# rarimo/ultragroth

Measured on AMD Instinct MI355X. Metric: proofs/s, higher is better.
Workload: dtype u32x9 (29-bit limbs, 254-bit modular integers)

## Files before the change

### ultragroth_amd/csrc/internal.hpp

```cpp
#pragma once
#include <hip/hip_runtime.h>
#include <cstdint>
#include <cstddef>
#include <vector>
#include "ec.hpp"
#include "stream_timer.hpp"

namespace ug {

Fr fr_root_of_unity(int s);
void bitrev_copy(u32* out, const u32* in, int logn, hipStream_t stream);

struct NttFusion {
    const u32* in2 = nullptr; u32* work = nullptr; const u32* fin_a = nullptr; const u32* fin_b = nullptr;
    u64 in2_stride = 0, work_stride = 0, fin_a_stride = 0, fin_b_stride = 0;
};

struct NttPass {
    const u32* in; u32* out; const u32* tw; const u32* post; const u32* post_const; const u32* in2; const u32* fin_a; const u32* fin_b;
    int logn, s0, k, j, gather_bitrev, scatter_bitrev;
    u64 in_stride, out_stride, in2_stride, fin_a_stride, fin_b_stride;
};
constexpr int NTT_MAX_PASSES = 8;

// ... 52 lines not shown
    void set_classes(const BucketClasses& k);
    void set_vectors(int v, u64 stride);
    u64 vector_count() const { return n / (u64)vectors; }
    int window_sets() const { return tables ? stride : windows; }
    int class_sets() const { return cls.on() ? (int)cls.cnt : 1; }
    int bucket_windows() const { return window_sets() * class_sets() * vectors; }
    u64 special_buckets() const { return cls.on() ? (u64)window_sets() * cls.specials : 0; }
    u64 total_buckets() const { return (u64)bucket_windows() * buckets + special_buckets(); }
    int result_points() const { return cls.on() ? 2 * bucket_windows() + (cls.specials ? window_sets() : 0) : bucket_windows(); }
    u64 expected_entries() const { return cls.on() ? ((n * (u64)windows) >> cls.q_log) * cls.cnt : n * (u64)windows; }
    DigitPlan digit_plan() const {
        DigitPlan d;
        d.n = n; d.c = c; d.windows = windows; d.buckets = buckets; d.sentinel = (u32)total_buckets(); d.tables = tables ? 1 : 0;
        d.set_map = 0; d.table_map = 0;
        if (tables)
            for (int w = 0; w < windows && w < 16; w++) { d.set_map |= (u64)(w % stride) << (4 * w); d.table_map |= (u64)(w / stride) << (4 * w); }
        d.q_log = cls.q_log; d.r0 = cls.r0; d.cnt = cls.on() ? cls.cnt : 1; d.specials = cls.on() ? cls.specials : 0;
        d.sp_lo = cls.sp_lo; d.sp_hi = cls.sp_hi; d.special_base = (u32)((u64)bucket_windows() * buckets);
        d.vec_count = (u32)vector_count(); d.vec_magic = 0; d.vec_shift = 0; d.vec_sets = (u32)window_sets(); d.vec_stride = vec_stride;
        if (vectors > 1) {
            int l = 0;
            while (((u64)1 << l) < (u64)d.vec_count) l++;
            d.vec_magic = (u32)((((u64)1 << 32) * (((u64)1 << l) - d.vec_count)) / d.vec_count + 1);
            d.vec_shift = l;
        }
        return d;
    }
};
constexpr int MSM_MAX_VECTORS = 16;
constexpr int TABLE_INDEX_BITS = 27;
constexpr int TABLE_MIN_C = 16, TABLE_MAX_C = 24;
double msm_model_cost(u64 n, int c, bool tables, int stride = 1);

struct HeavyBucket { u32 bucket, first_seg, last_seg, pad; };

int radix_plan(int bits, int* shift, int* bins_log);
void digit_pairs(const u32* scalars, const DigitPlan& plan, u32* keys, u32* vals, hipStream_t stream);
struct RadixSorter {
    u32* lookback = nullptr;
    u32* small = nullptr;
    u64 tiles_cap = 0;
    void reserve(u64 n_pairs, int ipt_min);
    void release();
    int sort(const u32* scalars, const MsmGeometry& geo, u32 sentinel, u64 n_pairs, int bits,
             u32* const buf_keys[2], u32* const buf_vals[2], u32* error_flag, hipStream_t stream, u32* n_valid_out = nullptr,
             bool* dropped_out = nullptr);
    ~RadixSorter() { release(); }
};

struct MsmSchedule {
    MsmGeometry geo;
    const u32* keys = nullptr;
    const u32* vals = nullptr;
    const u32* tkeys = nullptr;
    const u32* tvals = nullptr;
    u32* bucket_start = nullptr;
    u32* bucket_count = nullptr;
    u32* small_list = nullptr;
    int log_seg = 0;
    int log_seg_tail = 0;
    u32* heavy_list = nullptr;
    u32 heavy_cap = 0;
    u32* medium_list = nullptr;
    u32* heavy_offsets = nullptr;
    u32* meta = nullptr;
    u32 *keys_a = nullptr, *keys_b = nullptr, *vals_a = nullptr, *vals_b = nullptr;
    void* sort_tmp = nullptr; size_t sort_tmp_bytes = 0;
    RadixSorter sorter;
    u64 capacity_n = 0; u64 capacity_buckets = 0;
    void reserve(const MsmGeometry& g);
    void build(const u32* scalars_dev, const MsmGeometry& g, hipStream_t stream);
    void release();
    ~MsmSchedule() { release(); }
};

struct MsmWorkspace {
    u32* bucket_pts = nullptr;
    u32* chunk_pts = nullptr;
    u32* chunk_pts2 = nullptr;
    u32* slot_pts = nullptr;
    u32* task_pts = nullptr;
    size_t bucket_bytes = 0, chunk_bytes = 0, slot_bytes = 0, task_bytes = 0;
    void reserve(const MsmGeometry& g, bool g2, u64 n_segments, u32 n_heavy_tasks, int sets = 1);
    void release();
    ~MsmWorkspace() { release(); }
};

struct MsmPending {
    bool g2 = false;
    bool empty = true;
    int c = 0, window_sets = 0, class_sets = 1;
    int vectors = 1;
    BucketClasses cls;
    u32* host = nullptr;
};
constexpr int MSM_G2_PT_WORDS = 72;
constexpr size_t MSM_PENDING_WORDS = 128 * 72;
constexpr int MSM_QUEUE_DEPTH = 8;
constexpr int MSM_BATCH_WIDTH = 4;
struct MsmCall {
    struct Product { const u32* bases = nullptr; u64 n_bases = 0; int64_t delta = 0; u32* host = nullptr; };
    int count = 0;
    Product products[MSM_BATCH_WIDTH];
    int group = 0;
};
constexpr int MSM_PHASE_ALL = 0, MSM_PHASE_ACCUMULATE = 1, MSM_PHASE_TAIL = 2;
void msm_enqueue(bool g2, const MsmSchedule& s, MsmWorkspace& ws, const MsmCall& call, hipStream_t stream, LaunchTimer stats, MsmPending* pend,
                 int phase = MSM_PHASE_ALL);
// ... 61 lines not shown
```

### ultragroth_amd/csrc/msm.hip

```cpp
#ifdef UG_MEASURE
#include <hipcub/hipcub.hpp>
#endif
#include <algorithm>
#include <atomic>
#include <cstdlib>
#include <cstring>
#include <string>
#include <type_traits>
#include "dev_common.hpp"
#include "internal.hpp"
#include "segmap.hpp"

namespace ug {

namespace {

constexpr int LOG_SEG = 7;
constexpr u32 FIX_MAX = 32;
constexpr u32 MEDIUM_MAX = 4096;
constexpr u32 HEAVY_TASK = 1024;
constexpr int CHUNK = 32;

constexpr int ACC_BLOCK = 256;

typedef __attribute__((address_space(3))) u32 lds_u32;
template <class P> __device__ __forceinline__ void lds_get(Fp<P>& r, const lds_u32* p) {
#pragma unroll
    for (int i = 0; i < NL; i++) r.l[i] = p[i * ACC_BLOCK];
}
template <class P> __device__ __forceinline__ void lds_get(Fp2<P>& r, const lds_u32* p) { lds_get(r.a, p); lds_get(r.b, p + NL * ACC_BLOCK); }
template <class P> __device__ __forceinline__ void lds_set(lds_u32* p, const Fp<P>& v) {
#pragma unroll
    for (int i = 0; i < NL; i++) p[i * ACC_BLOCK] = v.l[i];
}
template <class P> __device__ __forceinline__ void lds_set(lds_u32* p, const Fp2<P>& v) { lds_set(p, v.a); lds_set(p + NL * ACC_BLOCK, v.b); }
template <class P> __device__ __forceinline__ u32 last_limb(const Fp<P>& v) { return v.l[NL - 1]; }
template <class P> __device__ __forceinline__ u32 last_limb(const Fp2<P>& v) { return v.b.l[NL - 1]; }
template <class F> struct TailLds {
    static constexpr int WORDS = sizeof(F) / sizeof(u32);
    static constexpr int AREA_WORDS = 2 * WORDS * ACC_BLOCK;
    lds_u32* slot;
    __device__ __forceinline__ lds_u32* after(const F& v) const {
        lds_u32* p = slot;
#if defined(__HIP_DEVICE_COMPILE__)
        asm volatile("" : "+v"(p) : "v"(last_limb(v)));
#endif
        return p;
    }
    __device__ __forceinline__ F zz() const { F r; lds_get(r, slot); return r; }
    __device__ __forceinline__ F zzz() const { F r; lds_get(r, slot + WORDS * ACC_BLOCK); return r; }
    __device__ __forceinline__ F zz_after(const F& v) const { F r; lds_get(r, after(v)); return r; }
    __device__ __forceinline__ F zzz_after(const F& v) const { F r; lds_get(r, after(v) + WORDS * ACC_BLOCK); return r; }
    __device__ __forceinline__ bool is_inf() const { return limbs_all_zero(zz()); }
    __device__ __forceinline__ void put(const F& zz, const F& zzz) { lds_set(slot, zz); lds_set(slot + WORDS * ACC_BLOCK, zzz); }
};

struct G1Cfg {
    typedef Fq F;
    typedef TailRegs<F> AccTail;
    static constexpr int AFF_WORDS = 16, PT_WORDS = 36, BLOCK = 256, ACC_WAVES = 3;
    static constexpr bool PREFETCH = true;
    static __device__ __forceinline__ bool load_affine(const u32* p, F& x, F& y) {
        u32 w[16];
        load8(w, p); load8(w + 8, p + 8);
        u32 o = 0;
#pragma unroll
        for (int i = 0; i < 16; i++) o |= w[i];
        if (o == 0) return false;
        x = unpack256<FqParams>(w); y = unpack256<FqParams>(w + 8);
        return true;
    }
    static __device__ __forceinline__ bool decode_affine(const u32* w, F& x, F& y) {
        u32 o = 0;
#pragma unroll
        for (int i = 0; i < 16; i++) o |= w[i];
        if (o == 0) return false;
        x = unpack256<FqParams>(w); y = unpack256<FqParams>(w + 8);
        return true;
    }
    static __device__ __forceinline__ void load_raw(u32* w, const u32* p) { load8(w, p); load8(w + 8, p + 8); }
    static __host__ __device__ __forceinline__ void store_affine_mont256(u32* o, const F& x, const F& y) {
        to_mont256(o, x); to_mont256(o + 8, y);
    }
    static __host__ __device__ __forceinline__ void store_affine_packed(u32* o, const F& x, const F& y) {
        pack256(o, cond_sub_q(mul(x, fp_one<FqParams>()))); pack256(o + 8, cond_sub_q(mul(y, fp_one<FqParams>())));
    }
    static __host__ __device__ __forceinline__ void to_words(u32* p, const XYZZ<F>& a, size_t stride) {
#pragma unroll
        for (int i = 0; i < NL; i++) {
            p[(size_t)i * stride] = a.x.l[i]; p[(size_t)(NL + i) * stride] = a.y.l[i];
            p[(size_t)(2 * NL + i) * stride] = a.zz.l[i]; p[(size_t)(3 * NL + i) * stride] = a.zzz.l[i];
        }
    }
    static __host__ __device__ __forceinline__ XYZZ<F> from_words(const u32* p, size_t stride) {
        XYZZ<F> a;
#pragma unroll
        for (int i = 0; i < NL; i++) {
            a.x.l[i] = p[(size_t)i * stride]; a.y.l[i] = p[(size_t)(NL + i) * stride];
            a.zz.l[i] = p[(size_t)(2 * NL + i) * stride]; a.zzz.l[i] = p[(size_t)(3 * NL + i) * stride];
        }
        return a;
    }
};
struct G2Cfg {
    typedef Fq2 F;
    typedef TailLds<F> AccTail;
    static constexpr int AFF_WORDS = 32, PT_WORDS = 72, BLOCK = 128, ACC_WAVES = 2;
    static constexpr bool PREFETCH = false;
    static __device__ __forceinline__ bool load_affine(const u32* p, F& x, F& y) {
        u32 w[32];
        load8(w, p); load8(w + 8, p + 8); load8(w + 16, p + 16); load8(w + 24, p + 24);
        u32 o = 0;
#pragma unroll
        for (int i = 0; i < 32; i++) o |= w[i];
        if (o == 0) return false;
        x.a = unpack256<FqParams>(w); x.b = unpack256<FqParams>(w + 8);
        y.a = unpack256<FqParams>(w + 16); y.b = unpack256<FqParams>(w + 24);
        return true;
    }
    static __device__ __forceinline__ bool decode_affine(const u32* w, F& x, F& y) {
        u32 o = 0;
#pragma unroll
        for (int i = 0; i < 32; i++) o |= w[i];
        if (o == 0) return false;
        x.a = unpack256<FqParams>(w); x.b = unpack256<FqParams>(w + 8);
        y.a = unpack256<FqParams>(w + 16); y.b = unpack256<FqParams>(w + 24);
        return true;
    }
    static __device__ __forceinline__ void load_raw(u32* w, const u32* p) {
        load8(w, p); load8(w + 8, p + 8); load8(w + 16, p + 16); load8(w + 24, p + 24);
    }
    static __host__ __device__ __forceinline__ void store_affine_mont256(u32* o, const F& x, const F& y) {
        to_mont256(o, x.a); to_mont256(o + 8, x.b); to_mont256(o + 16, y.a); to_mont256(o + 24, y.b);
    }
    static __host__ __device__ __forceinline__ void store_affine_packed(u32* o, const F& x, const F& y) {
        const Fq* f[4] = {&x.a, &x.b, &y.a, &y.b};
        for (int k = 0; k < 4; k++) pack256(o + 8 * k, cond_sub_q(mul(*f[k], fp_one<FqParams>())));
    }
    static __host__ __device__ __forceinline__ void to_words(u32* p, const XYZZ<F>& a, size_t stride) {
        const Fq* f[8] = {&a.x.a, &a.x.b, &a.y.a, &a.y.b, &a.zz.a, &a.zz.b, &a.zzz.a, &a.zzz.b};
#pragma unroll
        for (int k = 0; k < 8; k++)
#pragma unroll
            for (int i = 0; i < NL; i++) p[(size_t)(k * NL + i) * stride] = f[k]->l[i];
    }
    static __host__ __device__ __forceinline__ XYZZ<F> from_words(const u32* p, size_t stride) {
        XYZZ<F> a;
        Fq* f[8] = {&a.x.a, &a.x.b, &a.y.a, &a.y.b, &a.zz.a, &a.zz.b, &a.zzz.a, &a.zzz.b};
#pragma unroll
        for (int k = 0; k < 8; k++)
#pragma unroll
            for (int i = 0; i < NL; i++) f[k]->l[i] = p[(size_t)(k * NL + i) * stride];
        return a;
    }
};


__global__ void bucket_bounds_kernel(const u32* keys, u64 total_bound, u32 sentinel, u32* start, u32* count, u32* meta, int known) {
    const u64 total = known ? (u64)meta[1] : total_bound;
    const u64 p0 = ((u64)blockIdx.x * blockDim.x + threadIdx.x) * 4;
// ... 6 lines not shown
        for (int i = 0; i < 4; i++) k[1 + i] = p0 + i < total ? keys[p0 + i] : sentinel;
    }
    k[0] = p0 ? keys[p0 - 1] : sentinel;
    k[5] = p0 + 4 < total ? keys[p0 + 4] : sentinel;
#pragma unroll
    for (int i = 0; i < 4; i++) {
        const u64 p = p0 + i;
        const u32 key = k[1 + i];
        if (p >= total || key == sentinel) continue;
        if (p == 0 || k[i] != key) start[key] = (u32)p;
        if (k[2 + i] != key) count[key] = (u32)p + 1;
        if (k[2 + i] == sentinel) meta[1] = (u32)p + 1;
    }
}
__global__ __launch_bounds__(1024) void bucket_counts_kernel(u32* start, u32* count, u32 nb, int log_a, int log_b, u32* meta, u32* heavy_list,
                                                           u32* medium_list, u32 heavy_cap, u32* small_list) {
    __shared__ u32 listed, list_base;
    if (threadIdx.x == 0) listed = 0;
    __syncthreads();
    const u32 b = blockIdx.x * blockDim.x + threadIdx.x;
    u32 c = 0, first = 0, last = 0;
    if (b < nb) {
        const u32 e = count[b];
        c = e ? e - start[b] : 0;
        count[b] = c;
        if (c) { const SegMap map = SegMap::make(meta[1], log_a, log_b); first = map.seg_of(start[b]); last = map.seg_of(start[b] + c - 1); }
    }
    const u32 pieces = c ? last - first + 1 : 0;
    const bool small = pieces >= 2 && pieces <= FIX_MAX;
    u32 slot = 0;
    if (small) slot = atomicAdd(&listed, 1u);
    __syncthreads();
    if (threadIdx.x == 0 && listed) list_base = atomicAdd(&meta[4], listed);
    __syncthreads();
    if (small) small_list[list_base + slot] = b;
    if (pieces > MEDIUM_MAX) {
        u32 pos = atomicAdd(&meta[0], 1u);
        if (pos < heavy_cap) { heavy_list[4 * pos] = b; heavy_list[4 * pos + 1] = first; heavy_list[4 * pos + 2] = last; heavy_list[4 * pos + 3] = 0; }
    } else if (pieces > FIX_MAX) {
        u32 pos = atomicAdd(&meta[3], 1u);
        if (pos < heavy_cap) { medium_list[4 * pos] = b; medium_list[4 * pos + 1] = first; medium_list[4 * pos + 2] = last; medium_list[4 * pos + 3] = 0; }
    }
}

template <int I, int N> struct StaticFor {
    template <class Fn> static __device__ __forceinline__ void up(Fn&& f) { f(std::integral_constant<int, I>()); StaticFor<I + 1, N>::up(f); }
    template <class Fn> static __device__ __forceinline__ void down(Fn&& f) { StaticFor<I + 1, N>::down(f); f(std::integral_constant<int, I>()); }
};
template <int N> struct StaticFor<N, N> {
    template <class Fn> static __device__ __forceinline__ void up(Fn&&) {}
    template <class Fn> static __device__ __forceinline__ void down(Fn&&) {}
};

__global__ __launch_bounds__(1024) void transpose_entries_kernel(const u32* __restrict__ keys, const u32* __restrict__ vals,
                                                                const u32* __restrict__ meta, u32 sentinel, int log_a, int log_b,
                                                                u32* __restrict__ tkeys, u32* __restrict__ tvals) {
    extern __shared__ u32 tile[];
    const u32 n_valid = meta[1];
    const SegMap map = SegMap::make(n_valid, log_a, log_b);
    const u32 seg = blockIdx.x << 6;
    const u64 base = map.first_entry(seg);
    if (base >= n_valid) return;
    const int log_seg = map.log_len(seg);
    const u32 S = 1u << log_seg, row = S + 1;
    u32* tk = tile;
    u32* tv = tile + 64 * row;
    for (u32 i = threadIdx.x; i < (64u << log_seg); i += blockDim.x) {
        u64 src = base + i;
        bool in = src < n_valid;
        u32 sg = i >> log_seg, k = i & (S - 1);
        tk[sg * row + k] = in ? keys[src] : sentinel;
        tv[sg * row + k] = in ? vals[src] : 0u;
    }
    __syncthreads();
    for (u32 o = threadIdx.x; o < (64u << log_seg); o += blockDim.x) {
        u32 k = o >> 6, lane = o & 63;
        tkeys[base + o] = tk[lane * row + k];
        tvals[base + o] = tv[lane * row + k];
    }
}

template <class Cfg>
__global__ __launch_bounds__(ACC_BLOCK) __attribute__((amdgpu_waves_per_eu(Cfg::ACC_WAVES, Cfg::ACC_WAVES))) void segment_accumulate_kernel(const u32* __restrict__ bases, u64 n_bases, int64_t delta,
                                                                 const u32* __restrict__ keys, const u32* __restrict__ tkeys,
                                                                 const u32* __restrict__ tvals, const u32* __restrict__ meta, int log_a, int log_b,
                                                                 u32* __restrict__ bucket_pts, u32* __restrict__ slot_pts) {
    typedef typename Cfg::F F;
    const u32 n_valid = meta[1];
    const SegMap map = SegMap::make(n_valid, log_a, log_b);
    u32 t = blockIdx.x * blockDim.x + threadIdx.x;
    u64 lo = map.first_entry(t);
    if (lo >= n_valid) return;
    u64 hi = lo + ((u64)1 << map.log_len(t));
    if (hi > n_valid) hi = n_valid;
    const u32 cnt = (u32)(hi - lo);
    const u64 tbase = map.transposed(t, 0);
    u32 cur = tkeys[tbase];
    bool first_run = true;
    const bool start_open = lo > 0 && keys[lo - 1] == cur;
    F ax = field_zero((F*)0), ay = field_zero((F*)0);
    typename Cfg::AccTail tail;
    if constexpr (std::is_same<typename Cfg::AccTail, TailLds<F>>::value) {
        __shared__ u32 tail_area[TailLds<F>::AREA_WORDS];
        tail.slot = (lds_u32*)tail_area + threadIdx.x;
    }
    tail.put(field_zero((F*)0), field_zero((F*)0));
    auto store_acc = [&](u32* dst) {
        XYZZ<F> p;
        p.x = ax; p.y = ay; p.zz = tail.zz(); p.zzz = tail.zzz();
        Cfg::to_words(dst, p, 1);
    };
    const u32 IDX_MASK = (1u << TABLE_INDEX_BITS) - 1;
    auto close_run = [&](u32 key) {
        u32* dst = (first_run && start_open) ? slot_pts + (size_t)(2 * t) * Cfg::PT_WORDS : bucket_pts + (size_t)cur * Cfg::PT_WORDS;
        store_acc(dst);
        ax = field_zero((F*)0); ay = field_zero((F*)0);
        tail.put(field_zero((F*)0), field_zero((F*)0));
        cur = key;
        first_run = false;
    };
    if constexpr (Cfg::PREFETCH) {
        u32 raw[Cfg::AFF_WORDS];
        u32 nkey = cur, nval = tvals[tbase];
        int64_t nidx = (int64_t)(nval & IDX_MASK) + delta;
        bool nin = nidx >= 0 && (u64)nidx < n_bases;
        if (nin) Cfg::load_raw(raw, bases + ((u64)((nval >> TABLE_INDEX_BITS) & 15u) * n_bases + (u64)nidx) * Cfg::AFF_WORDS);
        for (u32 k = 0; k < cnt; k++) {
            F x, y;
            bool valid = nin && Cfg::decode_affine(raw, x, y);
            if (valid && (nval >> 31)) y = neg<1>(y);
            u32 key = nkey;
            if (k + 1 < cnt) {
                nkey = tkeys[tbase + ((u64)(k + 1) << 6)];
                nval = tvals[tbase + ((u64)(k + 1) << 6)];
                nidx = (int64_t)(nval & IDX_MASK) + delta;
                nin = nidx >= 0 && (u64)nidx < n_bases;
                if (nin) Cfg::load_raw(raw, bases + ((u64)((nval >> TABLE_INDEX_BITS) & 15u) * n_bases + (u64)nidx) * Cfg::AFF_WORDS);
            }
            if (key != cur) close_run(key);
            if (valid) xyzz_madd_at(ax, ay, tail, x, y);
        }
    } else {
        for (u32 k = 0; k < cnt; k++) {
            const u32 key = tkeys[tbase + ((u64)k << 6)], val = tvals[tbase + ((u64)k << 6)];
            const int64_t idx = (int64_t)(val & IDX_MASK) + delta;
            F x, y;
            bool valid = idx >= 0 && (u64)idx < n_bases &&
                         Cfg::load_affine(bases + ((u64)((val >> TABLE_INDEX_BITS) & 15u) * n_bases + (u64)idx) * Cfg::AFF_WORDS, x, y);
            if (valid && (val >> 31)) y = neg<1>(y);
            if (key != cur) close_run(key);
            if (valid) xyzz_madd_at(ax, ay, tail, x, y);
        }
    }
    const bool end_open = hi < n_valid && keys[hi] == cur;
    u32* dst;
    if (first_run && start_open) dst = slot_pts + (size_t)(2 * t) * Cfg::PT_WORDS;
    else if (end_open) dst = slot_pts + (size_t)(2 * t + 1) * Cfg::PT_WORDS;
    else dst = bucket_pts + (size_t)cur * Cfg::PT_WORDS;
    store_acc(dst);
}

#ifdef UG_MEASURE
#define UG_FOLD_PARAM , u32 fold_mask
#else
#define UG_FOLD_PARAM
#endif
template <int K>
__global__ __launch_bounds__(256) __attribute__((amdgpu_waves_per_eu(2, 2))) void segment_accumulate_group_kernel(
        const u32* __restrict__ bases, u64 n_slots, int64_t delta, const u32* __restrict__ keys, const u32* __restrict__ tkeys,
        const u32* __restrict__ tvals, const u32* __restrict__ meta, int log_a, int log_b, u32* __restrict__ bucket_pts,
        u32* __restrict__ slot_pts, size_t bucket_stride, size_t slot_stride UG_FOLD_PARAM) {
    typedef G1Cfg Cfg;
    typedef Fq F;
    const u32 n_valid = meta[1];
    const SegMap map = SegMap::make(n_valid, log_a, log_b);
    u32 t = blockIdx.x * blockDim.x + threadIdx.x;
    u64 lo = map.first_entry(t);
    if (lo >= n_valid) return;
    u64 hi = lo + ((u64)1 << map.log_len(t));
    if (hi > n_valid) hi = n_valid;
    const u32 cnt = (u32)(hi - lo);
    const u64 tbase = map.transposed(t, 0);
    u32 cur = tkeys[tbase];
    bool first_run = true;
    const bool start_open = lo > 0 && keys[lo - 1] == cur;
    XYZZ<F> acc[K];
    StaticFor<0, K>::up([&](auto m) { acc[m] = xyzz_inf<F>(); });
    const u32 IDX_MASK = (1u << TABLE_INDEX_BITS) - 1;
    auto record = [&](u32 val, int64_t idx, int m) -> const u32* {
#ifdef UG_MEASURE
        if (fold_mask != ~0u) return bases + (((u64)idx & fold_mask) * K + (u64)m) * Cfg::AFF_WORDS;
#endif
        return bases + (((u64)((val >> TABLE_INDEX_BITS) & 15u) * n_slots + (u64)idx) * K + (u64)m) * Cfg::AFF_WORDS;
    };
    auto flush = [&](bool to_slot, size_t slot, u32 bucket) {
        StaticFor<0, K>::up([&](auto m) {
            u32* dst = to_slot ? slot_pts + (size_t)m * slot_stride + slot * Cfg::PT_WORDS
                               : bucket_pts + (size_t)m * bucket_stride + (size_t)bucket * Cfg::PT_WORDS;
            Cfg::to_words(dst, acc[m], 1);
            acc[m] = xyzz_inf<F>();
        });
    };
    u32 raw[Cfg::AFF_WORDS];
    u32 nkey = cur, nval = tvals[tbase];
    int64_t nidx = (int64_t)(nval & IDX_MASK) + delta;
    bool nin = nidx >= 0 && (u64)nidx < n_slots;
    if (nin) Cfg::load_raw(raw, record(nval, nidx, 0));
    for (u32 k = 0; k < cnt; k++) {
        const u32 key = nkey, val = nval;
        const int64_t idx = nidx;
        const bool in = nin;
        const bool more = k + 1 < cnt;
        if (more) {
            nkey = tkeys[tbase + ((u64)(k + 1) << 6)];
            nval = tvals[tbase + ((u64)(k + 1) << 6)];
            nidx = (int64_t)(nval & IDX_MASK) + delta;
            nin = nidx >= 0 && (u64)nidx < n_slots;
        }
        if (key != cur) {
            flush(first_run && start_open, (size_t)2 * t, cur);
            cur = key;
            first_run = false;
        }
        StaticFor<0, K>::up([&](auto m) {
            F x, y;
            const bool valid = in && Cfg::decode_affine(raw, x, y);
            if (m + 1 < K) { if (in) Cfg::load_raw(raw, record(val, idx, m + 1)); }
            else if (more && nin) Cfg::load_raw(raw, record(nval, nidx, 0));
            if (valid && (val >> 31)) y = neg<1>(y);
            if (valid) acc[m] = xyzz_madd(acc[m], x, y);
        });
    }
    const bool end_open = hi < n_valid && keys[hi] == cur;
    if (first_run && start_open) flush(true, (size_t)2 * t, 0);
    else if (end_open) flush(true, (size_t)2 * t + 1, 0);
    else flush(false, 0, cur);
}

template <class Cfg>
__device__ __forceinline__ XYZZ<typename Cfg::F> load_piece(const u32* slot_pts, u32 first, u32 k) {
    size_t slot = k ? (size_t)2 * (first + k) : (size_t)2 * first + 1;
    return Cfg::from_words(slot_pts + slot * Cfg::PT_WORDS, 1);
}

template <class Cfg>
__global__ __launch_bounds__(128) void bucket_fixup_kernel(const u32* __restrict__ small_list, const u32* __restrict__ meta,
                                                           const u32* __restrict__ start, const u32* __restrict__ count, int log_a, int log_b,
                                                           const u32* __restrict__ slot_pts, u32* __restrict__ bucket_pts,
                                                           size_t slot_stride, size_t bucket_stride) {
    u32 t = blockIdx.x * blockDim.x + threadIdx.x;
    if (t >= meta[4]) return;
    slot_pts += blockIdx.y * slot_stride; bucket_pts += blockIdx.y * bucket_stride;
    typedef typename Cfg::F F;
    const u32 b = small_list[t];
    const u32 st = start[b];
    const SegMap map = SegMap::make(meta[1], log_a, log_b);
    const u32 first = map.seg_of(st), last = map.seg_of(st + count[b] - 1);
    const u32 pieces = last - first + 1;
    XYZZ<F> acc = load_piece<Cfg>(slot_pts, first, 0);
    for (u32 k = 1; k < pieces; k++) acc = xyzz_add(acc, load_piece<Cfg>(slot_pts, first, k));
    Cfg::to_words(bucket_pts + (size_t)b * Cfg::PT_WORDS, acc, 1);
}

template <class Cfg>
__device__ __forceinline__ XYZZ<typename Cfg::F> block_reduce(XYZZ<typename Cfg::F> acc, u32* lds) {
    const int tid = threadIdx.x, nth = Cfg::BLOCK;
    for (int stride = nth / 2; stride > 0; stride >>= 1) {
        if (tid >= stride && tid < 2 * stride) Cfg::to_words(lds + (tid - stride), acc, stride);
        __syncthreads();
        if (tid < stride) acc = xyzz_add(acc, Cfg::from_words(lds + tid, stride));
        __syncthreads();
    }
    return acc;
}

template <class Cfg>
__global__ __launch_bounds__(256) void medium_bucket_kernel(const HeavyBucket* mb, const u32* meta, u32 cap, const u32* slot_pts, u32* bucket_pts,
                                                            size_t slot_stride, size_t bucket_stride) {
    typedef typename Cfg::F F;
    slot_pts += blockIdx.y * slot_stride; bucket_pts += blockIdx.y * bucket_stride;
    const u32 lane = threadIdx.x & 63, n_waves = (gridDim.x * blockDim.x) >> 6;
    const u32 n_medium = meta[3] < cap ? meta[3] : cap;
    for (u32 wave = (blockIdx.x * blockDim.x + threadIdx.x) >> 6; wave < n_medium; wave += n_waves) {
        HeavyBucket h = mb[wave];
        u32 pieces = h.last_seg - h.first_seg + 1;
// ... 366 lines not shown
    if (g.n * (u64)g.windows > ((u64)1 << 30)) throw std::invalid_argument("msm: n * windows exceeds 2^30 entries");
    if (g.vector_count() > ((u64)1 << TABLE_INDEX_BITS)) throw std::invalid_argument("msm: more than 2^27 scalars in one schedule");
    geo = g;
    reserve(g);
    log_seg = segment_log(g.expected_entries());
    static const bool taper = !(getenv("UG_SEG_TAPER") && atoi(getenv("UG_SEG_TAPER")) == 0);
    log_seg_tail = (taper && log_seg == LOG_SEG && (g.expected_entries() >> log_seg) >= ((u64)1 << 16)) ? log_seg - 2 : log_seg;
    if (g.n == 0) return;
    u64 total = g.n * g.windows;
    u32 nb = (u32)g.total_buckets();
    u32 sentinel = nb;
    int end_bit = 1;
    while (((u64)1 << end_bit) <= sentinel) end_bit++;
    UG_HIP(hipMemsetAsync(meta, 0, 32, stream));
#ifdef UG_MEASURE
    static const bool use_cub = getenv("UG_SORT") && !strcmp(getenv("UG_SORT"), "cub");
#else
    constexpr bool use_cub = false;
#endif
    const bool pairs_first = use_cub || g.windows > 16;
    bool dropped = false;
    if (pairs_first) digit_pairs(scalars_dev, g.digit_plan(), keys_a, vals_a, stream);
#ifdef UG_MEASURE
    if (use_cub) {
        hipcub::DoubleBuffer<u32> dk(keys_a, keys_b), dv(vals_a, vals_b);
        if (!sort_tmp_bytes) {
            size_t need = 0;
            UG_HIP(hipcub::DeviceRadixSort::SortPairs(nullptr, need, dk, dv, (int)total, 0, 32));
            epoch_alloc(sort_tmp, need); sort_tmp_bytes = need;
        }
        size_t tmp = sort_tmp_bytes;
        UG_HIP(hipcub::DeviceRadixSort::SortPairs(sort_tmp, tmp, dk, dv, (int)total, 0, end_bit, stream));
        keys = dk.Current();
        vals = dv.Current();
    } else
#endif
    {
        u32* const bk[2] = {keys_a, keys_b};
        u32* const bv[2] = {vals_a, vals_b};
        const int at = sorter.sort(pairs_first ? nullptr : scalars_dev, g, sentinel, total, end_bit, bk, bv, meta + 7, stream, meta + 1, &dropped);
        keys = bk[at];
        vals = bv[at];
    }
    UG_HIP(hipMemsetAsync(bucket_start, 0, (size_t)nb * 4, stream));
    UG_HIP(hipMemsetAsync(bucket_count, 0, (size_t)nb * 4, stream));
    hipLaunchKernelGGL(bucket_bounds_kernel, dim3((unsigned)((total + 1023) / 1024)), dim3(256), 0, stream,
                       keys, total, sentinel, bucket_start, bucket_count, meta, dropped ? 1 : 0);
    UG_KERNEL_CHECK();
    hipLaunchKernelGGL(bucket_counts_kernel, dim3((nb + 1023) / 1024), dim3(1024), 0, stream, bucket_start, bucket_count, nb,
                       log_seg, log_seg_tail, meta, heavy_list, medium_list, heavy_cap, small_list);
    UG_KERNEL_CHECK();
    hipLaunchKernelGGL(heavy_plan_kernel, dim3(1), dim3(1024), 0, stream, (const HeavyBucket*)heavy_list, heavy_cap, meta, heavy_offsets);
    UG_KERNEL_CHECK();
    u64 n_tiles = (SegMap::max_segments(total, log_seg, log_seg_tail) + 63) / 64;
    u32* tk = (keys == keys_a) ? keys_b : keys_a;
    u32* tv = (vals == vals_a) ? vals_b : vals_a;
    {
        size_t lds = (size_t)2 * 64 * (((size_t)1 << log_seg) + 1) * 4;
        hipLaunchKernelGGL(transpose_entries_kernel, dim3((unsigned)n_tiles), dim3(1024), lds, stream,
                           keys, vals, meta, sentinel, log_seg, log_seg_tail, tk, tv);
        UG_KERNEL_CHECK();
    }
    tkeys = tk; tvals = tv;
}

void MsmSchedule::release() {
    dev_free(keys_a); dev_free(keys_b); dev_free(vals_a); dev_free(vals_b); dev_free(sort_tmp);
    dev_free(bucket_start); dev_free(bucket_count); dev_free(small_list); dev_free(heavy_list); dev_free(medium_list); dev_free(heavy_offsets); dev_free(meta);
    sorter.release();
    capacity_n = capacity_buckets = 0; sort_tmp_bytes = 0; vals = nullptr; keys = nullptr; heavy_cap = 0;
}

void MsmWorkspace::reserve(const MsmGeometry& g, bool g2, u64 n_segments, u32 n_heavy_tasks, int sets) {
    size_t ptw = (size_t)(g2 ? G2Cfg::PT_WORDS : G1Cfg::PT_WORDS) * (size_t)sets;
    size_t need = (size_t)g.total_buckets() * ptw * 4;
    if (need > bucket_bytes) { epoch_alloc(bucket_pts, need); bucket_bytes = need; }
    const int chunk = reduce_chunk(g, sets, g2);
    size_t cneed = ((size_t)(g.cls.on() ? 2 : 1) * g.bucket_windows() * (g.buckets / chunk) + (size_t)g.window_sets()) * ptw * 4;
    if (cneed > chunk_bytes) { epoch_alloc(chunk_pts, cneed); epoch_alloc(chunk_pts2, cneed); chunk_bytes = cneed; }
    size_t sneed = (size_t)n_segments * 2 * ptw * 4;
    if (sneed > slot_bytes) { epoch_alloc(slot_pts, sneed); slot_bytes = sneed; }
    size_t tneed = (size_t)n_heavy_tasks * ptw * 4;
    if (tneed > task_bytes) { epoch_alloc(task_pts, tneed); task_bytes = tneed; }
}
void MsmWorkspace::release() {
    dev_free(bucket_pts); dev_free(chunk_pts); dev_free(chunk_pts2); dev_free(slot_pts); dev_free(task_pts);
    bucket_bytes = chunk_bytes = slot_bytes = task_bytes = 0;
}

namespace {
template <class Cfg>
void msm_enqueue_multi(const MsmSchedule& s, MsmWorkspace& ws, const MsmCall& call, hipStream_t stream, LaunchTimer stats, MsmPending* pend, int phase) {
    const int count = call.count, group = call.group;
    const MsmCall::Product* const p = call.products;
    const bool do_acc = phase != MSM_PHASE_TAIL, do_tail = phase != MSM_PHASE_ACCUMULATE;
    typedef typename Cfg::F F;
    const MsmGeometry& g = s.geo;
    if (count < 1 || count > MSM_BATCH_WIDTH) throw std::logic_error("msm: batch size");
    int live[MSM_BATCH_WIDTH], k = 0;
    for (int j = 0; j < count; j++) {
        pend[j] = MsmPending();
        pend[j].g2 = Cfg::PT_WORDS == G2Cfg::PT_WORDS;
        pend[j].c = g.c; pend[j].window_sets = g.window_sets(); pend[j].class_sets = g.class_sets(); pend[j].cls = g.cls; pend[j].vectors = g.vectors;
        pend[j].host = p[j].host;
        if (g.n == 0 || p[group ? 0 : j].n_bases == 0) continue;
        if ((size_t)g.result_points() * Cfg::PT_WORDS > MSM_PENDING_WORDS - 1) throw std::logic_error("msm: result block too large");
        pend[j].empty = false;
        live[k++] = j;
    }
    if (!k) return;
    const u64 total = g.n * g.windows;
    const u64 nseg = SegMap::max_segments(total, s.log_seg, s.log_seg_tail);
    const u32 heavy_max = (u32)std::min<u64>(s.heavy_cap, nseg / MEDIUM_MAX + 1);
    const u32 tasks_max = (u32)((nseg + heavy_max) / HEAVY_TASK + heavy_max + 1);
    const u32 medium_max = (u32)std::min<u64>(s.heavy_cap, nseg / (FIX_MAX - 1) + 1);
    if (do_acc) ws.reserve(g, Cfg::PT_WORDS == G2Cfg::PT_WORDS, nseg, tasks_max, k);
    const size_t bucket_stride = (size_t)g.total_buckets() * Cfg::PT_WORDS, slot_stride = (size_t)nseg * 2 * Cfg::PT_WORDS,
                 task_stride = (size_t)tasks_max * Cfg::PT_WORDS;
    if constexpr (Cfg::PT_WORDS == G1Cfg::PT_WORDS) {
        if (group && do_acc) {
#ifdef UG_MEASURE
            const char* fold = getenv("UG_GROUP_FOLD_LOG");
            const u32 fold_mask = fold && *fold ? ((1u << atoi(fold)) - 1) : ~0u;
#define UG_FOLD_ARG , fold_mask
#else
#define UG_FOLD_ARG
#endif
            StreamTimer::Scope timed = stats.time(stream, g.n * g.windows * (u64)group);
            if (nseg) {
                const dim3 grid((unsigned)((nseg + 255) / 256)), block(256);
#define UG_GROUP_LAUNCH(K_) hipLaunchKernelGGL((segment_accumulate_group_kernel<K_>), grid, block, 0, stream, p[0].bases, p[0].n_bases, \
                                                   p[0].delta, s.keys, s.tkeys, s.tvals, s.meta, s.log_seg, s.log_seg_tail, ws.bucket_pts, ws.slot_pts,   \
                                                   bucket_stride, slot_stride UG_FOLD_ARG)
                if (group == 3) UG_GROUP_LAUNCH(3);
                else if (group == 2) UG_GROUP_LAUNCH(2);
                else throw std::logic_error("msm: group size");
#undef UG_GROUP_LAUNCH
#undef UG_FOLD_ARG
                UG_KERNEL_CHECK();
            }
            timed.stop();
        }
    } else if (group) throw std::logic_error("msm: groups are G1 only");
    for (int q = 0; q < (group || !do_acc ? 0 : k); q++) {
        const int j = live[q];
        StreamTimer::Scope timed = stats.time(stream, g.n * g.windows);
        if (nseg) {
            hipLaunchKernelGGL(segment_accumulate_kernel<Cfg>, dim3((unsigned)((nseg + ACC_BLOCK - 1) / ACC_BLOCK)), dim3(ACC_BLOCK), 0, stream,
                               p[j].bases, p[j].n_bases, p[j].delta, s.keys, s.tkeys, s.tvals, s.meta, s.log_seg, s.log_seg_tail,
                               ws.bucket_pts + q * bucket_stride, ws.slot_pts + q * slot_stride);
            UG_KERNEL_CHECK();
        }
        timed.stop();
    }
    if (!do_tail) return;
    if (nseg > 1) {
        const u64 small_max = std::min<u64>(g.total_buckets(), nseg);
        hipLaunchKernelGGL(bucket_fixup_kernel<Cfg>, dim3((unsigned)((small_max + 127) / 128), k), dim3(128), 0, stream,
                           s.small_list, s.meta, s.bucket_start, s.bucket_count, s.log_seg, s.log_seg_tail, ws.slot_pts, ws.bucket_pts,
                           slot_stride, bucket_stride);
        UG_KERNEL_CHECK();
        if (nseg > FIX_MAX) {
            hipLaunchKernelGGL(medium_bucket_kernel<Cfg>, dim3(std::min<u32>((medium_max + 3) / 4, 2048), k), dim3(256), 0, stream,
                               (const HeavyBucket*)s.medium_list, s.meta, medium_max, ws.slot_pts, ws.bucket_pts, slot_stride, bucket_stride);
            UG_KERNEL_CHECK();
        }
        if (nseg > MEDIUM_MAX) {
            hipLaunchKernelGGL(heavy_partial_kernel<Cfg>, dim3(tasks_max, k), dim3(Cfg::BLOCK), 0, stream,
                               (const HeavyBucket*)s.heavy_list, s.heavy_offsets, s.meta, heavy_max, ws.slot_pts, ws.task_pts,
                               slot_stride, task_stride);
            UG_KERNEL_CHECK();
            hipLaunchKernelGGL(heavy_final_kernel<Cfg>, dim3(heavy_max, k), dim3(Cfg::BLOCK), 0, stream,
                               (const HeavyBucket*)s.heavy_list, s.heavy_offsets, s.meta, heavy_max, ws.task_pts, ws.bucket_pts,
                               task_stride, bucket_stride);
            UG_KERNEL_CHECK();
        }
    }
    int chunk = reduce_chunk(g, k, Cfg::PT_WORDS == G2Cfg::PT_WORDS);
    const int windows = g.bucket_windows();
    const int bw = windows * k;
    const bool classes = g.cls.on();
    u32 cpw = g.buckets / chunk;
    u32 nchunks = cpw * bw;
    hipLaunchKernelGGL(bucket_chunk_reduce_kernel<Cfg>, dim3((nchunks + 127) / 128), dim3(128), 0, stream,
                       ws.bucket_pts, s.bucket_count, g.buckets, chunk, nchunks, g.c, ws.chunk_pts, (u32)windows,
                       classes ? ws.chunk_pts + (size_t)nchunks * Cfg::PT_WORDS : (u32*)nullptr, (size_t)g.total_buckets());
    UG_KERNEL_CHECK();
    const int tree_sets = classes ? 2 * bw : bw;
    u32* cur = ws.chunk_pts; u32* nxt = ws.chunk_pts2;
    while (cpw > 1) {
        if ((u64)(cpw / 16) * tree_sets >= 8192) {
            const int group = 16;
            u32 n_out = (cpw / group) * tree_sets;
            hipLaunchKernelGGL(ec_sum_groups_kernel<Cfg>, dim3((n_out + 127) / 128), dim3(128), 0, stream, cur, nxt, n_out, group);
            cpw /= group;
        } else {
            const int group = cpw >= 256 ? 256 : (int)cpw;
            u32 n_out = (cpw / group) * tree_sets;
            hipLaunchKernelGGL(ec_sum_wave_kernel<Cfg>, dim3((n_out + 3) / 4), dim3(256), 0, stream, cur, nxt, n_out, group);
            cpw /= group;
        }
        UG_KERNEL_CHECK();
// ... 130 lines not shown
```

### ultragroth_amd/csrc/segmap.hpp

```cpp
#pragma once
#include "ff.hpp"

namespace ug {

struct SegMap {
    u32 split, seg0;
    int log_a, log_b;
    UG_HD static SegMap make(u64 n_valid, int log_a, int log_b) {
        SegMap m;
        m.log_a = log_a; m.log_b = log_b;
        const u64 tile = (u64)64 << log_a;
        const u64 split = log_b < log_a ? ((n_valid - (n_valid >> 3)) / tile) * tile : ((n_valid + tile - 1) / tile) * tile;
        m.split = (u32)split; m.seg0 = (u32)(split >> log_a);
        return m;
    }
    UG_HD u32 seg_of(u32 pos) const { return pos < split ? pos >> log_a : seg0 + ((pos - split) >> log_b); }
    UG_HD u32 first_entry(u32 seg) const { return seg < seg0 ? seg << log_a : split + ((seg - seg0) << log_b); }
    UG_HD int log_len(u32 seg) const { return seg < seg0 ? log_a : log_b; }
    UG_HD u64 transposed(u32 seg, u32 k) const {
        const u64 tile0 = seg < seg0 ? (u64)(seg >> 6) << (log_a + 6) : (u64)split + ((u64)((seg - seg0) >> 6) << (log_b + 6));
        return tile0 + ((u64)k << 6) + (seg & 63);
    }
    static inline u64 max_segments(u64 total, int log_a, int log_b) {
        if (log_b >= log_a) return (total + ((u64)1 << log_a) - 1) >> log_a;
        return (total >> log_a) + (((total >> 3) + ((u64)64 << log_a)) >> log_b) + 64;
    }
};

}
```

Baseline: 7.892.

## Replace global transpose pass with per-wave LDS staging of segment entries

Measured after the change: 7.907 (median of 2 runs). About the same (+0.2%).

```diff
diff --git a/ultragroth_amd/csrc/internal.hpp b/ultragroth_amd/csrc/internal.hpp
--- a/ultragroth_amd/csrc/internal.hpp
+++ b/ultragroth_amd/csrc/internal.hpp
@@ -128,8 +128,6 @@
     MsmGeometry geo;
     const u32* keys = nullptr;
     const u32* vals = nullptr;
-    const u32* tkeys = nullptr;
-    const u32* tvals = nullptr;
     u32* bucket_start = nullptr;
     u32* bucket_count = nullptr;
     u32* small_list = nullptr;
diff --git a/ultragroth_amd/csrc/msm.hip b/ultragroth_amd/csrc/msm.hip
--- a/ultragroth_amd/csrc/msm.hip
+++ b/ultragroth_amd/csrc/msm.hip
@@ -60,6 +60,7 @@
     typedef TailRegs<F> AccTail;
     static constexpr int AFF_WORDS = 16, PT_WORDS = 36, BLOCK = 256, ACC_WAVES = 3;
     static constexpr bool PREFETCH = true;
+    static constexpr u32 STAGE_R = 8;
     static __device__ __forceinline__ bool load_affine(const u32* p, F& x, F& y) {
         u32 w[16];
         load8(w, p); load8(w + 8, p + 8);
@@ -106,6 +107,7 @@
     typedef Fq2 F;
     typedef TailLds<F> AccTail;
     static constexpr int AFF_WORDS = 32, PT_WORDS = 72, BLOCK = 128, ACC_WAVES = 2;
+    static constexpr u32 STAGE_R = 8;
     static constexpr bool PREFETCH = false;
     static __device__ __forceinline__ bool load_affine(const u32* p, F& x, F& y) {
         u32 w[32];
@@ -218,52 +220,86 @@
     template <class Fn> static __device__ __forceinline__ void down(Fn&&) {}
 };
 
-__global__ __launch_bounds__(1024) void transpose_entries_kernel(const u32* __restrict__ keys, const u32* __restrict__ vals,
-                                                                const u32* __restrict__ meta, u32 sentinel, int log_a, int log_b,
-                                                                u32* __restrict__ tkeys, u32* __restrict__ tvals) {
-    extern __shared__ u32 tile[];
+template <u32 R> struct EntryStage {
+    typedef SegStage<R> St;
+    static constexpr int AREA_WORDS = 2 * (int)St::AREA * (ACC_BLOCK / 64);
+    lds_u32* row;
+    u32 area_first;
+    u32 seg_first;
+    int log_len;
+    __device__ __forceinline__ void refill(u32* area, const u32* __restrict__ keys, const u32* __restrict__ vals, u32 n_valid, u32 sentinel, u32 k0) const {
+        __builtin_amdgcn_fence(__ATOMIC_RELEASE, "wavefront");
+        __builtin_amdgcn_wave_barrier();
+        u32 lane = threadIdx.x & 63;
+#if defined(__HIP_DEVICE_COMPILE__)
+        asm volatile("" : "+v"(lane));
+#endif
+#pragma unroll
+        for (u32 pass = 0; pass < St::PASSES; pass++) {
+            const u32 pos = (u32)St::load_pos(seg_first, log_len, k0, lane, pass);
+            uint4 a = make_uint4(sentinel, sentinel, sentinel, sentinel), b = make_uint4(0u, 0u, 0u, 0u);
+            if (pos < n_valid) {
+                a = *reinterpret_cast<const uint4*>(keys + pos);
+                b = *reinterpret_cast<const uint4*>(vals + pos);
+                if (pos + 1 >= n_valid) { a.y = sentinel; b.y = 0u; }
+                if (pos + 2 >= n_valid) { a.z = sentinel; b.z = 0u; }
+                if (pos + 3 >= n_valid) { a.w = sentinel; b.w = 0u; }
+            }
+            lds_u32* dk = (lds_u32*)area + area_first + St::cell(St::load_seg(lane, pass), St::load_off(lane));
+            dk[0] = a.x; dk[1] = a.y; dk[2] = a.z; dk[3] = a.w;
+            lds_u32* dv = dk + St::AREA;
+            dv[0] = b.x; dv[1] = b.y; dv[2] = b.z; dv[3] = b.w;
+        }
+        __builtin_amdgcn_fence(__ATOMIC_RELEASE, "wavefront");
+        __builtin_amdgcn_wave_barrier();
+        __builtin_amdgcn_fence(__ATOMIC_ACQUIRE, "wavefront");
+    }
+    __device__ __forceinline__ u32 key(u32 k) const { return row[k & (R - 1)]; }
+    __device__ __forceinline__ u32 val(u32 k) const { return row[St::AREA + (k & (R - 1))]; }
+};
+
+struct LaneWalk {
+    u32 t;
+    u32 wcnt;
+    u32 cnt;
+    u32 lo;
+};
+template <u32 R>
+__device__ __forceinline__ bool lane_walk(LaneWalk& w, EntryStage<R>& stage, u32* area, const SegMap& map, u32 n_valid) {
+    w.t = blockIdx.x * blockDim.x + threadIdx.x;
+    const u32 lane = threadIdx.x & 63;
+    const u32 wlo = __builtin_amdgcn_readfirstlane(map.first_entry(w.t - lane));
+    if (wlo >= n_valid) return false;
+    const int log_len = __builtin_amdgcn_readfirstlane(map.log_len(w.t));
+    const u32 len = 1u << log_len;
+    w.wcnt = n_valid - wlo < len ? n_valid - wlo : len;
+    w.lo = wlo + (lane << log_len);
+    w.cnt = w.lo >= n_valid ? 0u : (n_valid - w.lo < len ? n_valid - w.lo : len);
+    stage.area_first = __builtin_amdgcn_readfirstlane((threadIdx.x >> 6) * (2 * SegStage<R>::AREA));
+    stage.row = (lds_u32*)area + stage.area_first + SegStage<R>::cell(lane, 0);
+    stage.seg_first = wlo; stage.log_len = log_len;
+    return true;
+}
+
+template <class Cfg>
+__global__ __launch_bounds__(ACC_BLOCK) __attribute__((amdgpu_waves_per_eu(Cfg::ACC_WAVES, Cfg::ACC_WAVES))) void segment_accumulate_kernel(const u32* __restrict__ bases, u64 n_bases, int64_t delta,
+                                                                 const u32* __restrict__ keys, const u32* __restrict__ vals,
+                                                                 const u32* __restrict__ meta, u32 sentinel, int log_a, int log_b,
+                                                                 u32* __restrict__ bucket_pts, u32* __restrict__ slot_pts) {
+    typedef typename Cfg::F F;
     const u32 n_valid = meta[1];
     const SegMap map = SegMap::make(n_valid, log_a, log_b);
-    const u32 seg = blockIdx.x << 6;
-    const u64 base = map.first_entry(seg);
-    if (base >= n_valid) return;
-    const int log_seg = map.log_len(seg);
-    const u32 S = 1u << log_seg, row = S + 1;
-    u32* tk = tile;
-    u32* tv = tile + 64 * row;
-    for (u32 i = threadIdx.x; i < (64u << log_seg); i += blockDim.x) {
-        u64 src = base + i;
-        bool in = src < n_valid;
-        u32 sg = i >> log_seg, k = i & (S - 1);
-        tk[sg * row + k] = in ? keys[src] : sentinel;
-        tv[sg * row + k] = in ? vals[src] : 0u;
-    }
-    __syncthreads();
-    for (u32 o = threadIdx.x; o < (64u << log_seg); o += blockDim.x) {
-        u32 k = o >> 6, lane = o & 63;
-        tkeys[base + o] = tk[lane * row + k];
-        tvals[base + o] = tv[lane * row + k];
-    }
-}
-
-template <class Cfg>
-__global__ __launch_bounds__(ACC_BLOCK) __attribute__((amdgpu_waves_per_eu(Cfg::ACC_WAVES, Cfg::ACC_WAVES))) void segment_accumulate_kernel(const u32* __restrict__ bases, u64 n_bases, int64_t delta,
-                                                                 const u32* __restrict__ keys, const u32* __restrict__ tkeys,
-                                                                 const u32* __restrict__ tvals, const u32* __restrict__ meta, int log_a, int log_b,
-                                                                 u32* __restrict__ bucket_pts, u32* __restrict__ slot_pts) {
-    typedef typename Cfg::F F;
-    const u32 n_valid = meta[1];
-    const SegMap map = SegMap::make(n_valid, log_a, log_b);
-    u32 t = blockIdx.x * blockDim.x + threadIdx.x;
-    u64 lo = map.first_entry(t);
-    if (lo >= n_valid) return;
-    u64 hi = lo + ((u64)1 << map.log_len(t));
-    if (hi > n_valid) hi = n_valid;
-    const u32 cnt = (u32)(hi - lo);
-    const u64 tbase = map.transposed(t, 0);
-    u32 cur = tkeys[tbase];
+    __shared__ u32 stage_area[EntryStage<Cfg::STAGE_R>::AREA_WORDS];
+    EntryStage<Cfg::STAGE_R> stage;
+    LaneWalk w;
+    if (!lane_walk(w, stage, stage_area, map, n_valid)) return;
+    auto refill = [&](u32 k0) { stage.refill(stage_area, keys, vals, n_valid, sentinel, k0); };
+    refill(0);
+    const u32 t = w.t, cnt = w.cnt, wcnt = w.wcnt;
+    const bool live = cnt != 0;
+    u32 cur = stage.key(0);
     bool first_run = true;
-    const bool start_open = lo > 0 && keys[lo - 1] == cur;
+    const bool start_open = live && w.lo > 0 && keys[w.lo - 1] == cur;
     F ax = field_zero((F*)0), ay = field_zero((F*)0);
     typename Cfg::AccTail tail;
     if constexpr (std::is_same<typename Cfg::AccTail, TailLds<F>>::value) {
@@ -287,37 +323,44 @@
     };
     if constexpr (Cfg::PREFETCH) {
         u32 raw[Cfg::AFF_WORDS];
-        u32 nkey = cur, nval = tvals[tbase];
+        u32 nkey = cur, nval = stage.val(0);
         int64_t nidx = (int64_t)(nval & IDX_MASK) + delta;
-        bool nin = nidx >= 0 && (u64)nidx < n_bases;
+        bool nin = live && nidx >= 0 && (u64)nidx < n_bases;
         if (nin) Cfg::load_raw(raw, bases + ((u64)((nval >> TABLE_INDEX_BITS) & 15u) * n_bases + (u64)nidx) * Cfg::AFF_WORDS);
-        for (u32 k = 0; k < cnt; k++) {
+        for (u32 k = 0; k < wcnt; k++) {
+            const bool mine = k < cnt;
             F x, y;
-            bool valid = nin && Cfg::decode_affine(raw, x, y);
+            bool valid = mine && nin && Cfg::decode_affine(raw, x, y);
             if (valid && (nval >> 31)) y = neg<1>(y);
             u32 key = nkey;
+            if (((k + 1) & (Cfg::STAGE_R - 1)) == 0 && k + 1 < wcnt) refill(k + 1);
             if (k + 1 < cnt) {
-                nkey = tkeys[tbase + ((u64)(k + 1) << 6)];
-                nval = tvals[tbase + ((u64)(k + 1) << 6)];
+                nkey = stage.key(k + 1);
+                nval = stage.val(k + 1);
                 nidx = (int64_t)(nval & IDX_MASK) + delta;
                 nin = nidx >= 0 && (u64)nidx < n_bases;
                 if (nin) Cfg::load_raw(raw, bases + ((u64)((nval >> TABLE_INDEX_BITS) & 15u) * n_bases + (u64)nidx) * Cfg::AFF_WORDS);
             }
-            if (key != cur) close_run(key);
+            if (mine && key != cur) close_run(key);
             if (valid) xyzz_madd_at(ax, ay, tail, x, y);
         }
     } else {
-        for (u32 k = 0; k < cnt; k++) {
-            const u32 key = tkeys[tbase + ((u64)k << 6)], val = tvals[tbase + ((u64)k << 6)];
-            const int64_t idx = (int64_t)(val & IDX_MASK) + delta;
-            F x, y;
-            bool valid = idx >= 0 && (u64)idx < n_bases &&
-                         Cfg::load_affine(bases + ((u64)((val >> TABLE_INDEX_BITS) & 15u) * n_bases + (u64)idx) * Cfg::AFF_WORDS, x, y);
-            if (valid && (val >> 31)) y = neg<1>(y);
-            if (key != cur) close_run(key);
-            if (valid) xyzz_madd_at(ax, ay, tail, x, y);
-        }
-    }
+        for (u32 k = 0; k < wcnt; k++) {
+            if (k && (k & (Cfg::STAGE_R - 1)) == 0) refill(k);
+            if (k < cnt) {
+                const u32 key = stage.key(k), val = stage.val(k);
+                const int64_t idx = (int64_t)(val & IDX_MASK) + delta;
+                F x, y;
+                bool valid = idx >= 0 && (u64)idx < n_bases &&
+                             Cfg::load_affine(bases + ((u64)((val >> TABLE_INDEX_BITS) & 15u) * n_bases + (u64)idx) * Cfg::AFF_WORDS, x, y);
+                if (valid && (val >> 31)) y = neg<1>(y);
+                if (key != cur) close_run(key);
+                if (valid) xyzz_madd_at(ax, ay, tail, x, y);
+            }
+        }
+    }
+    if (!live) return;
+    const u32 hi = w.lo + cnt;
     const bool end_open = hi < n_valid && keys[hi] == cur;
     u32* dst;
     if (first_run && start_open) dst = slot_pts + (size_t)(2 * t) * Cfg::PT_WORDS;
@@ -333,23 +376,24 @@
 #endif
 template <int K>
 __global__ __launch_bounds__(256) __attribute__((amdgpu_waves_per_eu(2, 2))) void segment_accumulate_group_kernel(
-        const u32* __restrict__ bases, u64 n_slots, int64_t delta, const u32* __restrict__ keys, const u32* __restrict__ tkeys,
-        const u32* __restrict__ tvals, const u32* __restrict__ meta, int log_a, int log_b, u32* __restrict__ bucket_pts,
+        const u32* __restrict__ bases, u64 n_slots, int64_t delta, const u32* __restrict__ keys, const u32* __restrict__ vals,
+        const u32* __restrict__ meta, u32 sentinel, int log_a, int log_b, u32* __restrict__ bucket_pts,
         u32* __restrict__ slot_pts, size_t bucket_stride, size_t slot_stride UG_FOLD_PARAM) {
     typedef G1Cfg Cfg;
     typedef Fq F;
     const u32 n_valid = meta[1];
     const SegMap map = SegMap::make(n_valid, log_a, log_b);
-    u32 t = blockIdx.x * blockDim.x + threadIdx.x;
-    u64 lo = map.first_entry(t);
-    if (lo >= n_valid) return;
-    u64 hi = lo + ((u64)1 << map.log_len(t));
-    if (hi > n_valid) hi = n_valid;
-    const u32 cnt = (u32)(hi - lo);
-    const u64 tbase = map.transposed(t, 0);
-    u32 cur = tkeys[tbase];
+    __shared__ u32 stage_area[EntryStage<Cfg::STAGE_R>::AREA_WORDS];
+    EntryStage<Cfg::STAGE_R> stage;
+    LaneWalk w;
+    if (!lane_walk(w, stage, stage_area, map, n_valid)) return;
+    auto refill = [&](u32 k0) { stage.refill(stage_area, keys, vals, n_valid, sentinel, k0); };
+    refill(0);
+    const u32 t = w.t, cnt = w.cnt, wcnt = w.wcnt;
+    const bool live = cnt != 0;
+    u32 cur = stage.key(0);
     bool first_run = true;
-    const bool start_open = lo > 0 && keys[lo - 1] == cur;
+    const bool start_open = live && w.lo > 0 && keys[w.lo - 1] == cur;
     XYZZ<F> acc[K];
     StaticFor<0, K>::up([&](auto m) { acc[m] = xyzz_inf<F>(); });
     const u32 IDX_MASK = (1u << TABLE_INDEX_BITS) - 1;
@@ -368,22 +412,23 @@
         });
     };
     u32 raw[Cfg::AFF_WORDS];
-    u32 nkey = cur, nval = tvals[tbase];
+    u32 nkey = cur, nval = stage.val(0);
     int64_t nidx = (int64_t)(nval & IDX_MASK) + delta;
-    bool nin = nidx >= 0 && (u64)nidx < n_slots;
+    bool nin = live && nidx >= 0 && (u64)nidx < n_slots;
     if (nin) Cfg::load_raw(raw, record(nval, nidx, 0));
-    for (u32 k = 0; k < cnt; k++) {
+    for (u32 k = 0; k < wcnt; k++) {
         const u32 key = nkey, val = nval;
         const int64_t idx = nidx;
-        const bool in = nin;
+        const bool in = k < cnt && nin;
         const bool more = k + 1 < cnt;
+        if (((k + 1) & (Cfg::STAGE_R - 1)) == 0 && k + 1 < wcnt) refill(k + 1);
         if (more) {
-            nkey = tkeys[tbase + ((u64)(k + 1) << 6)];
-            nval = tvals[tbase + ((u64)(k + 1) << 6)];
+            nkey = stage.key(k + 1);
+            nval = stage.val(k + 1);
             nidx = (int64_t)(nval & IDX_MASK) + delta;
             nin = nidx >= 0 && (u64)nidx < n_slots;
         }
-        if (key != cur) {
+        if (k < cnt && key != cur) {
             flush(first_run && start_open, (size_t)2 * t, cur);
             cur = key;
             first_run = false;
@@ -397,6 +442,8 @@
             if (valid) acc[m] = xyzz_madd(acc[m], x, y);
         });
     }
+    if (!live) return;
+    const u32 hi = w.lo + cnt;
     const bool end_open = hi < n_valid && keys[hi] == cur;
     if (first_run && start_open) flush(true, (size_t)2 * t, 0);
     else if (end_open) flush(true, (size_t)2 * t + 1, 0);
@@ -869,16 +916,6 @@
     UG_KERNEL_CHECK();
     hipLaunchKernelGGL(heavy_plan_kernel, dim3(1), dim3(1024), 0, stream, (const HeavyBucket*)heavy_list, heavy_cap, meta, heavy_offsets);
     UG_KERNEL_CHECK();
-    u64 n_tiles = (SegMap::max_segments(total, log_seg, log_seg_tail) + 63) / 64;
-    u32* tk = (keys == keys_a) ? keys_b : keys_a;
-    u32* tv = (vals == vals_a) ? vals_b : vals_a;
-    {
-        size_t lds = (size_t)2 * 64 * (((size_t)1 << log_seg) + 1) * 4;
-        hipLaunchKernelGGL(transpose_entries_kernel, dim3((unsigned)n_tiles), dim3(1024), lds, stream,
-                           keys, vals, meta, sentinel, log_seg, log_seg_tail, tk, tv);
-        UG_KERNEL_CHECK();
-    }
-    tkeys = tk; tvals = tv;
 }
 
 void MsmSchedule::release() {
@@ -947,7 +984,7 @@
             if (nseg) {
                 const dim3 grid((unsigned)((nseg + 255) / 256)), block(256);
 #define UG_GROUP_LAUNCH(K_) hipLaunchKernelGGL((segment_accumulate_group_kernel<K_>), grid, block, 0, stream, p[0].bases, p[0].n_bases, \
-                                                   p[0].delta, s.keys, s.tkeys, s.tvals, s.meta, s.log_seg, s.log_seg_tail, ws.bucket_pts, ws.slot_pts,   \
+                                                   p[0].delta, s.keys, s.vals, s.meta, (u32)g.total_buckets(), s.log_seg, s.log_seg_tail, ws.bucket_pts, ws.slot_pts,   \
                                                    bucket_stride, slot_stride UG_FOLD_ARG)
                 if (group == 3) UG_GROUP_LAUNCH(3);
                 else if (group == 2) UG_GROUP_LAUNCH(2);
@@ -964,7 +1001,7 @@
         StreamTimer::Scope timed = stats.time(stream, g.n * g.windows);
         if (nseg) {
             hipLaunchKernelGGL(segment_accumulate_kernel<Cfg>, dim3((unsigned)((nseg + ACC_BLOCK - 1) / ACC_BLOCK)), dim3(ACC_BLOCK), 0, stream,
-                               p[j].bases, p[j].n_bases, p[j].delta, s.keys, s.tkeys, s.tvals, s.meta, s.log_seg, s.log_seg_tail,
+                               p[j].bases, p[j].n_bases, p[j].delta, s.keys, s.vals, s.meta, (u32)g.total_buckets(), s.log_seg, s.log_seg_tail,
                                ws.bucket_pts + q * bucket_stride, ws.slot_pts + q * slot_stride);
             UG_KERNEL_CHECK();
         }
diff --git a/ultragroth_amd/csrc/segmap.hpp b/ultragroth_amd/csrc/segmap.hpp
--- a/ultragroth_amd/csrc/segmap.hpp
+++ b/ultragroth_amd/csrc/segmap.hpp
@@ -27,4 +27,19 @@
     }
 };
 
+template <u32 R> struct SegStage {
+    static_assert(R >= 4 && R <= 32 && (R & (R - 1)) == 0, "SegStage: R");
+    static constexpr u32 ROW = R + 1;
+    static constexpr u32 AREA = 64 * ROW;
+    static constexpr u32 LANES = R / 4;
+    static constexpr u32 PASSES = R / 4;
+    static constexpr u32 SEGS = 64 / LANES;
+    UG_HD static u32 cell(u32 s, u32 k) { return s * ROW + (k & (R - 1)); }
+    UG_HD static u32 load_seg(u32 lane, u32 pass) { return pass * SEGS + lane / LANES; }
+    UG_HD static u32 load_off(u32 lane) { return (lane % LANES) * 4; }
+    UG_HD static u64 load_pos(u64 seg_first, int log_len, u32 k0, u32 lane, u32 pass) {
+        return seg_first + ((u64)load_seg(lane, pass) << log_len) + k0 + load_off(lane);
+    }
+};
+
 }
```
